# ioloizou/g1_locomotion

Hardware: AMD Instinct MI355X
Metric: QP solves/sec, SRBD N=10 12-state/12-input (higher is better)
Workload: dtype f64; 1 GPU; configs[1]: batch=4096/GPU random SRBD states, N=10, 2-contact alternating single support friction cone, fp64; tails deferred (SRBDQP_FLAG_DEFER_TAIL: the ~4 % of a batch that reach a rho-restart mark finish in the next launch on their stream; srbdqp_flush inside the timed region, every batch complete when the clock stops); steps rotate over 4 distinct device batches; horizon=10, batch_per_gpu=4096, kernel=wave_defer_f64_n10_s2, streams=2, longest_first_hint=False, deferred_tails=True, world_size=1, distinct_batches=4, max_iter=250, rho_restart_iter=0, rho_restart_count=0, set_up_dtype=f64

## Files before the change

g1_locomotion_amd/csrc/srbdqp_setup1.hpp:

```cpp
#pragma once
#include "srbdqp_split.hpp"

namespace srbdqp {

#ifdef SRBDQP_WAVE_STAMPS
#define WSTAMP(a, b, idx) SRBDQP_STAMP(a, b, idx)
#define WSTAMP_RT(a, b, idx) do { if ((a).stamps && threadIdx.x == 0) (a).stamps[(size_t)(b) * 16 + (idx)] = (long long)__builtin_amdgcn_s_memrealtime(); } while (0)
#else
#define WSTAMP(a, b, idx) do { } while (0)
#define WSTAMP_RT(a, b, idx) do { } while (0)
#endif

template <int N, int MAXS>
struct Setup1Smem {
    using S = CompactSmem<N, MAXS>;
    static constexpr int n = Dims<N>::n;
    static constexpr int up2(int v) { return (v + 1) & ~1; }
    static constexpr int o_x0 = S::o_x0, o_tm = S::o_tm, o_J = S::o_J;
    static constexpr int o_cp = S::o_R;
    static constexpr int o_mt = o_cp + up2(9 * N);
    static constexpr int o_ab = o_mt + 18 * N;
    static constexpr int o_gv = o_mt + up2(9 * S::NPAIR);
    static constexpr int o_t1 = o_gv + up2(9 * N);
    static constexpr int o_t2 = o_t1 + up2(9 * N);
    static constexpr int o_x0c = o_t1;
    static constexpr int o_tf = o_x0c + up2(S::nmax) + 16;
    static constexpr int endT = (o_t2 + up2(9 * N) > o_tf + 6 * N) ? o_t2 + up2(9 * N) : o_tf + 6 * N;
    static constexpr int o_xref = up2(endT);
    static constexpr int o_foot = o_xref + up2(N * 13);
    static constexpr int o_pcom = o_foot + N * 12;
    static constexpr int o_eh = o_foot;
    static constexpr int o_gx = o_foot;
    static constexpr int o_scr = o_xref;
    static constexpr int endIn = o_pcom + up2(N * 3);
    static constexpr int endIn2 = (endIn > o_scr + 258) ? endIn : o_scr + 258;
    static constexpr int kStgRow = 18;
    static constexpr int kStgTile = 16 * kStgRow;
    static constexpr int endStg = (endIn2 > o_cp + S::NT * kStgTile) ? endIn2 : o_cp + S::NT * kStgTile;
    static constexpr int endAb = o_ab + 16 * S::NT * kAbStride;
    static constexpr int o_end = endStg > endAb ? endStg : endAb;
    static constexpr size_t bytes = (size_t)o_end * sizeof(double);
    static constexpr int kPairs = S::NPAIR;
    static constexpr int kPairSlots = (N / 2) * N + N;
    static constexpr int o_pd = o_t1;
    static constexpr int o_pq = up2(endIn);
    static constexpr bool pairs_fit = N % 2 == 0 && kPairs <= 64 && 2 * kPairSlots <= 2 * up2(9 * N) && o_pq + 4 * kPairSlots <= o_end;
    static constexpr bool supported = SplitWs<N, MAXS>::supported && S::NT <= 4;
    static_assert(!supported || pairs_fit, "a lane and an LDS slot for every step pair of a horizon the one-wave kernel takes");
    static_assert(n + 6 * N <= o_end - o_eh || true, "");
};

template <int N, int MAXS, bool FUSED, bool DUMP, bool PHI, int RP>
__device__ __forceinline__ bool setup1_pass(const KArgs& a, const QpIo& io, const int b, double* sm, double& rho_b, int& rs_pass, int& rs_done) {
    using S = CompactSmem<N, MAXS>;
    using W = SplitWs<N, MAXS>;
    using L1 = Setup1Smem<N, MAXS>;
    constexpr int n = Dims<N>::n, m = Dims<N>::m, NT = S::NT;
    int lane = threadIdx.x;
    if constexpr (RP == 2) asm volatile("" : "+v"(lane));
    [[maybe_unused]] double* const park = sm + L1::o_end;
    int mcol = lane & 15, kq = lane >> 4;
    double* ws = FUSED ? nullptr : a.ws + (size_t)b * W::doubles;
    int* icnt = reinterpret_cast<int*>(sm + S::o_int);
    int* imisc = icnt + 2 * N;
    uint8_t* act = reinterpret_cast<uint8_t*>(imisc + 8);
    uint8_t* sct = reinterpret_cast<uint8_t*>(sm + S::o_ct);
    const double* SQ = sm + S::o_sq;
    const double* CP = sm + L1::o_cp;

    WSTAMP(a, b, 0);
    WSTAMP_RT(a, b, 12);
    constexpr int JT = (12 * N + 63) / 64;
    double yc, ys;
    [[maybe_unused]] double v_xr[JT];
    if constexpr (RP == 2) {
        const int k = lane < N ? lane : 0;
        yc = sm[S::o_tm + k * 9 + 0];
        ys = sm[S::o_tm + k * 9 + 1];
    } else {
        const double* gx0 = io.x0 + (size_t)b * 13;
        const double* gxr = io.xref + (size_t)b * N * 13;
        const double* gft = io.foot + (size_t)b * N * 12;
        const uint8_t* gct = io.contact + (size_t)b * N * 4;
        const double* gpc = io.pcom ? io.pcom + (size_t)b * N * 3 : nullptr;
        const double v_x0 = gx0[lane < 13 ? lane : 0];
        const uint8_t v_ct = gct[lane < 4 * N ? lane : 0];
        const double v_yaw = gxr[(lane < N ? lane : 0) * 13 + 2];
        double v_f[JT][3], v_p[JT][3];
#pragma unroll
        for (int t = 0; t < JT; ++t) {
            const int tt = (lane + 64 * t < 12 * N) ? lane + 64 * t : 0;
            const int k = tt / 12, ci = (tt % 12) / 3;
            const double* pc = gpc ? gpc + k * 3 : gxr + k * 13 + 3;
#pragma unroll
            for (int c = 0; c < 3; ++c) { v_f[t][c] = gft[k * 12 + 3 * ci + c]; v_p[t][c] = pc[c]; }
            v_xr[t] = gxr[k * 13 + (tt - 12 * k)];
        }
        sincos(v_yaw, &ys, &yc);
        if (lane < 13) sm[S::o_x0 + lane] = v_x0;
        if (lane >= 32 && lane < 44) sm[S::o_sq + lane - 32] = a.sqrtq[lane - 32];
        if (lane < N * 4) sct[lane] = v_ct ? 1 : 0;
        if (lane < N) {
            double* T = sm + S::o_tm + lane * 9;
            T[0] = yc;  T[1] = ys;  T[2] = 0.0;
            T[3] = -ys; T[4] = yc;  T[5] = 0.0;
            T[6] = 0.0; T[7] = 0.0; T[8] = 1.0;
        }
        {
            const bool flag = (lane < 4 * N) && v_ct != 0;
            const unsigned long long bal = __ballot(flag);
            if (flag) act[__popcll(bal & ((1ull << lane) - 1ull))] = (uint8_t)lane;
            if (lane < N) icnt[lane] = __popcll(bal & ((4 * (lane + 1) >= 64) ? ~0ull : ((1ull << (4 * (lane + 1))) - 1ull)));
            const bool over = lane < N && __popcll((bal >> (4 * (lane < N ? lane : 0))) & 0xFull) > MAXS;
            const unsigned long long viol = __ballot(over);
            if (lane == 0) {
                imisc[0] = __popcll(bal);
                imisc[1] = viol != 0ull;
                sm[S::o_misc] = 0.0;
                sm[S::o_misc + 1] = 0.0;
            }
        }
#pragma unroll
        for (int t = 0; t < JT; ++t) {
            const int tt = lane + 64 * t;
            const int k = (tt < 12 * N ? tt : 0) / 12, cc = tt - 12 * k, ax = cc % 3;
            const double cs = __shfl(yc, k), sn = __shfl(ys, k);
            const double i0 = a.iinv[0], i1 = a.iinv[1], i2 = a.iinv[2];
            const double w00 = cs * cs * i0 + sn * sn * i1, w01 = cs * sn * (i0 - i1), w11 = sn * sn * i0 + cs * cs * i1;
            const double rx = v_f[t][0] - v_p[t][0];
            const double ry = v_f[t][1] - v_p[t][1];
            const double rz = v_f[t][2] - v_p[t][2];
            const double s0 = (ax == 0) ? 0.0 : ((ax == 1) ? -rz : ry);
            const double s1 = (ax == 0) ? rz : ((ax == 1) ? 0.0 : -rx);
            const double s2 = (ax == 0) ? -ry : ((ax == 1) ? rx : 0.0);
            if (tt < 12 * N) {
                double* J = sm + S::o_J + k * 36;
                J[0 * 12 + cc] = w00 * s0 + w01 * s1;
                J[1 * 12 + cc] = w01 * s0 + w11 * s1;
                J[2 * 12 + cc] = i2 * s2;
            }
        }
    }
    double ccm = 0.0, csm = 0.0;
#pragma unroll
    for (int k = 0; k < N; ++k) {
        const double c = lane_bcast(yc, k), s = lane_bcast(ys, k);
        ccm += (k <= lane) ? c : 0.0;
        csm += (k <= lane) ? s : 0.0;
    }
    if (lane < N) {
        double* C = sm + L1::o_cp + lane * 9;
        C[0] = ccm;  C[1] = csm; C[2] = 0.0;
        C[3] = -csm; C[4] = ccm; C[5] = 0.0;
        C[6] = 0.0;  C[7] = 0.0; C[8] = (double)(lane + 1);
    }
    __syncthreads();
    const int na = imisc[0];
    const int n_eff = 3 * na;
    double* xs0 = sm + L1::o_mt;
    static_assert(L1::o_end - L1::o_mt >= n + 12 * N, "early-exit scratch");
    if (RP != 2 && (imisc[1] != 0 || na == 0)) {
        if constexpr (DUMP) { if (lane == 0) a.ub_out[(size_t)b * m] = (imisc[1] != 0) ? -1.0 : 0.0; return false; }
        for (int c = lane; c < n; c += 64) xs0[c] = 0.0;
        if (io.y_out) for (int i = lane; i < m; i += 64) io.y_out[(size_t)b * m + i] = 0.0;
        if (lane == 0) {
            if (io.status) io.status[b] = (imisc[1] != 0) ? kStatusContactBound : 1;
            if (io.iters) io.iters[b] = a.iters_base;
            if constexpr (!FUSED) ws[S::o_misc + 1] = 1.0;
        }
        __syncthreads();
        rollout_and_store_to<N, S, 64>(a, io.u_out, io.x_out, b, sm, xs0, xs0 + n);
        return false;
    }

    WSTAMP(a, b, 1);
    const double dt = a.dt, dt2 = a.dt * a.dt, dtm = a.dt * a.inv_mass, dt2m = dt2 * a.inv_mass;
    double* DE = sm + L1::o_mt;
    double* GV = sm + L1::o_gv;
    if constexpr (RP != 2) {
#pragma unroll
        for (int t = 0; t < JT; ++t) {
            const int k = lane + 64 * t;
            const int kc = k < n ? k : 0, i = kc / 12, kk = kc - 12 * i;
            const double v = SQ[kk] * (free_response_sel<N, L1>(a, sm, i, kk) - v_xr[t]);
            if (k < n) sm[L1::o_eh + k] = v;
        }
    }
    const int pair_c = lane < L1::kPairs ? lane : L1::kPairs - 1;
    const int pair_r = pair_c / (N + 1), pair_k = pair_c - pair_r * (N + 1);
    const bool pair_lo = pair_k < N - pair_r;
    const int pair_m = pair_lo ? pair_r : N - 1 - pair_r, pair_i = pair_m + (pair_lo ? pair_k : pair_k - (N - pair_r));
    const double pair_da = CP[9 * pair_i] - CP[9 * pair_m], pair_db = CP[9 * pair_i + 1] - CP[9 * pair_m + 1];
    double* PD = sm + L1::o_pd;
    double* PQ = sm + L1::o_pq;
    {
        const double w0 = SQ[0] * SQ[0], w1 = SQ[1] * SQ[1], w2 = SQ[2] * SQ[2];
        const double da = pair_da, db = pair_db, dz = (double)(pair_i - pair_m);
        if (lane < L1::kPairs) {
            PD[2 * lane] = da;
            PD[2 * lane + 1] = db;
            PQ[4 * lane] = fma(w0 * da, da, (w1 * db) * db);
            PQ[4 * lane + 1] = fma(w0 * da, db, -((w1 * db) * da));
            PQ[4 * lane + 2] = fma(w0 * db, db, (w1 * da) * da);
            PQ[4 * lane + 3] = (pair_i == N - 1) ? 0.0 : (w2 * dz) * dz;
        }
    }
    __syncthreads();
    const int pair_base = (2 * lane < N) ? lane * (N + 1) : (N - lane) * N;
    if (lane < N) {
        const int mm = lane;
        double t1a = 0.0, t1b = 0.0, t2aa = 0.0, t2ab = 0.0, t2bb = 0.0, t2zz = 0.0;
#pragma unroll
        for (int s = 0; s < N; ++s) {
            if (s < N - mm) {
                const double* pd = PD + 2 * (pair_base + s);
                const double* pq = PQ + 4 * (pair_base + s);
                t1a += pd[0];
                t1b += pd[1];
                t2aa += pq[0];
                t2ab += pq[1];
                t2bb += pq[2];
                t2zz += pq[3];
            }
        }
        const double dzl = (double)(N - 1 - mm);
        t2zz = fma((SQ[2] * SQ[2]) * dzl, dzl, t2zz);
        const double t1z = (double)(((N - mm) * (N - mm - 1)) / 2);
        const double Cm[9] = {ccm, csm, 0.0, -csm, ccm, 0.0, 0.0, 0.0, (double)(mm + 1)};
        const double t1[9] = {t1a, t1b, 0.0, -t1b, t1a, 0.0, 0.0, 0.0, t1z};
        const double t2[9] = {t2aa, t2ab, 0.0, t2ab, t2bb, 0.0, 0.0, 0.0, t2zz};
        de_step<N>(Cm, t1, t2, SQ, dt2, mm, DE + 18 * mm);
    }
    auto gt_tables = [&](const double* vec) {
        {
            const double* v = vec + 12 * pair_i;
            const double p0 = SQ[0] * v[0], p1 = SQ[1] * v[1], p2 = SQ[2] * v[2], dz = (double)(pair_i - pair_m);
            if (lane < L1::kPairs) {
                PQ[4 * lane] = fma(dt, SQ[6] * v[6], dt2 * fma(pair_da, p0, (-pair_db) * p1));
                PQ[4 * lane + 1] = fma(dt, SQ[7] * v[7], dt2 * fma(pair_db, p0, pair_da * p1));
                PQ[4 * lane + 2] = fma(dt, SQ[8] * v[8], dt2 * (dz * p2));
            }
        }
        __syncthreads();
        if (lane < 3 * N) {
            const int j = lane / 3, comp = lane - 3 * j;
            const double* pq = PQ + 4 * ((2 * j < N) ? j * (N + 1) : (N - j) * N) + comp;
            double acc = 0.0;
#pragma unroll
            for (int s = 0; s < N; ++s)
                if (s < N - j) acc += pq[4 * s];
            GV[9 * j + comp] = acc;
        }
        static_assert(6 * N <= 64, "the force entries of the G'v tables are one trip of the wave");
        if (lane < 6 * N) {
            const int j = lane / 6, comp = 3 + (lane - 6 * j);
            const double* v = vec + 12 * j + ((comp < 6) ? comp : 3 + comp);
            const double winc = (comp < 6) ? 1.0 : 0.0;
            double acc = 0.0, w = (comp < 6) ? 0.0 : 1.0;
#pragma unroll
            for (int s = 0; s < N; ++s) {
                if (s < N - j) {
                    double term = w * v[12 * s];
                    asm volatile("" : "+v"(term));
                    acc += term;
                }
                w += winc;
            }
            GV[9 * j + comp] = acc;
        }
    };
    auto gt_eval = [&](int c) -> double {
        const int e = c / 3, ax = c - 3 * e, gc = act[e], j = gc >> 2;
        const double* J = sm + S::o_J + j * 36 + 3 * (gc & 3) + ax;
        const double* g = GV + 9 * j;
        return a.s * (J[0] * g[0] + J[12] * g[1] + J[24] * g[2] + SQ[3 + ax] * dt2m * g[3 + ax] + SQ[9 + ax] * dtm * g[6 + ax]);
    };
    __syncthreads();
    if constexpr (RP != 2) gt_tables(sm + L1::o_eh);
    __syncthreads();
    WSTAMP(a, b, 2);
    if constexpr (RP != 2) for (int c = lane; c < n_eff; c += 64) sm[S::o_q + c] = gt_eval(c);
    if (RP >= 2 || a.warm_u) {
        double* TF = sm + L1::o_tf;
        for (int c = lane; c < n_eff; c += 64)
            sm[L1::o_x0c + c] = (RP >= 2 ? park[c] : a.warm_u[(size_t)b * n + 3 * act[c / 3] + (c % 3)]) / a.s;
        __syncthreads();
        for (int tt = lane; tt < 6 * N; tt += 64) {
            const int j = tt / 6, comp = tt - 6 * j;
            double acc = 0.0;
            for (int e = (j ? icnt[j - 1] : 0); e < icnt[j]; ++e) {
                const double* x = sm + L1::o_x0c + 3 * e;
                if (comp < 3) {
                    const double* J = sm + S::o_J + j * 36 + comp * 12 + 3 * (act[e] & 3);
                    acc += J[0] * x[0] + J[1] * x[1] + J[2] * x[2];
                } else {
                    acc += x[comp - 3];
                }
            }
            TF[tt] = acc;
        }
        __syncthreads();
        for (int k = lane; k < n; k += 64) {
            const int i = k / 12, kk = k - 12 * i;
            const double acc = gx_row<N>(CP, TF, i, kk, dt, dt2, dtm, dt2m);
            sm[L1::o_gx + k] = SQ[kk] * a.s * acc;
        }
        __syncthreads();
        gt_tables(sm + L1::o_gx);
        __syncthreads();
        for (int c = lane; c < n_eff; c += 64) sm[S::o_px0 + c] = gt_eval(c) + a.rs2 * sm[L1::o_x0c + c];
    } else {
        for (int c = lane; c < n_eff; c += 64) sm[S::o_px0 + c] = 0.0;
    }

    if constexpr (PHI) {
        double* phi = ws + W::o_phi;
        const double x0_keep = (lane < 13) ? sm[S::o_x0 + lane] : 0.0;
        for (int kc = 0; kc < 13; ++kc) {
            __syncthreads();
            if (lane < 13) sm[S::o_x0 + lane] = (lane == kc) ? 1.0 : 0.0;
            __syncthreads();
            for (int k = lane; k < n; k += 64) {
                const int i = k / 12, kk = k - 12 * i;
                sm[L1::o_eh + k] = SQ[kk] * free_response<N, L1>(a, sm, i, kk);
            }
            __syncthreads();
            gt_tables(sm + L1::o_eh);
            __syncthreads();
            for (int c = lane; c < n_eff; c += 64) phi[c * 13 + kc] = gt_eval(c);
        }
        __syncthreads();
        if (lane < 13) sm[S::o_x0 + lane] = x0_keep;
        __syncthreads();
    }
    WSTAMP(a, b, 3);
    v4d Kt[NT][NT];
    __syncthreads();
    {
        double* AB = sm + L1::o_ab;
        kasm_rows<N>(sm + S::o_J, CP, DE, SQ, act, n_eff, a.s, dt2m, dtm, AB, lane, 64, 16 * NT);
        __syncthreads();
        typedef double d2 __attribute__((ext_vector_type(2)));
        const double dgxy = uni(a.rs2 + a.sigma + 2.0 * rho_b), dgz = uni(a.rs2 + a.sigma + (4.0 * a.mu * a.mu + a.rho_fz) * rho_b);
        const int d3 = (mcol - kq + 3) % 3;
        const double ind[3] = {d3 == 0 ? 1.0 : 0.0, d3 == 1 ? 1.0 : 0.0, d3 == 2 ? 1.0 : 0.0};
        double eqd[4];
#pragma unroll
        for (int q = 0; q < 4; ++q) eqd[q] = (kq + 4 * q == mcol) ? 1.0 : 0.0;
        double Bv[NT][8], dcol[NT];
#pragma unroll
        for (int tb = 0; tb < NT; ++tb) {
            const int c = 16 * tb + mcol;
            const d2* row = reinterpret_cast<const d2*>(AB + kAbStride * c + 8);
#pragma unroll
            for (int i = 0; i < 4; ++i) { const d2 v = row[i]; Bv[tb][2 * i] = v[0]; Bv[tb][2 * i + 1] = v[1]; }
            dcol[tb] = (c < n_eff) ? (((tb + mcol) % 3 < 2) ? dgxy : dgz) : 1.0;
        }
#pragma unroll
        for (int ta = 0; ta < NT; ++ta) {
#pragma unroll
            for (int q = 0; q < 4; ++q) {
                const int r = 16 * ta + kq + 4 * q;
                const d2* row = reinterpret_cast<const d2*>(AB + kAbStride * r);
                double Av[8];
#pragma unroll
                for (int i = 0; i < 4; ++i) { const d2 v = row[i]; Av[2 * i] = v[0]; Av[2 * i + 1] = v[1]; }
#pragma unroll
                for (int tb = ta; tb < NT; ++tb) {
                    double v = Av[0] * Bv[tb][0];
#pragma unroll
                    for (int i = 1; i < 6; ++i) v = fma(Av[i], Bv[tb][i], v);
                    const double ft = fma(Av[7], Bv[tb][7], Av[6] * Bv[tb][6]);
                    v = fma(ind[((ta + q - tb) % 3 + 3) % 3], ft, v);
                    if (ta == tb) v = fma(eqd[q], dcol[tb], v);
                    Kt[ta][tb][q] = v;
                }
            }
        }
    }
    __syncthreads();
    WSTAMP(a, b, 4);
    WSTAMP(a, b, 5);
    if constexpr (DUMP) {
        dump_presolved<N>(a, b, n_eff, na, sm + S::o_q, act, [&](auto&& put) {
#pragma unroll
            for (int ta = 0; ta < NT; ++ta)
#pragma unroll
                for (int tb = ta; tb < NT; ++tb)
#pragma unroll
                    for (int q = 0; q < 4; ++q)
                        if (16 * ta + kq + 4 * q <= 16 * tb + mcol) put(16 * ta + kq + 4 * q, 16 * tb + mcol, Kt[ta][tb][q]);
        });
        return false;
    }

    double* scr = sm + L1::o_scr;
    auto a_operand_read = [&](double (&op)[4]) {
#pragma unroll
        for (int r = 0; r < 4; ++r) op[r] = scr[mcol * 16 + ((4 * r + kq) ^ mcol)];
        asm volatile("" ::: "memory");
    };
    auto a_operand = [&](const v4d& x, double (&op)[4]) {
        asm volatile("" ::: "memory");
#pragma unroll
        for (int q = 0; q < 4; ++q) {
            const int row = kq + 4 * q;
            scr[row * 16 + (mcol ^ row)] = x[q];
        }
        asm volatile("" ::: "memory");
        a_operand_read(op);
    };
    const v4d zero4 = (v4d){0.0, 0.0, 0.0, 0.0};

    bool all_ok = true;
#pragma unroll
    for (int j = 0; j < NT; ++j) {
        bool ok;
        const v4d w = diag16_invert_dpp_packed(Kt[j][j], lane, ok, scr);
        all_ok = all_ok && ok;
        Kt[j][j] = w;
        if (j + 1 < NT) {
            double wa[4];
            a_operand_read(wa);
#pragma unroll
            for (int bb = j + 1; bb < NT; ++bb) {
                v4d o = zero4;
#pragma unroll
                for (int r = 0; r < 4; ++r) o = mfma_f64(wa[r], Kt[j][bb][r], o);
                Kt[j][bb] = o;
            }
#pragma unroll
            for (int aa = j + 1; aa < NT; ++aa)
#pragma unroll
                for (int bb = aa; bb < NT; ++bb)
#pragma unroll
                    for (int r = 0; r < 4; ++r) Kt[aa][bb] = mfma_f64(-Kt[j][aa][r], Kt[j][bb][r], Kt[aa][bb]);
        }
    }
    if (!all_ok && lane == 0) sm[S::o_misc] = 1.0;
    WSTAMP(a, b, 6);

#pragma unroll
    for (int i = 1; i < NT; ++i) {
        double wa[4];
        a_operand(Kt[i][i], wa);
#pragma unroll
        for (int j = 0; j < i; ++j) {
            v4d sacc = zero4;
#pragma unroll
            for (int k = j; k < i; ++k) {
                const v4d& wkj = (k == j) ? Kt[j][j] : Kt[j][k];
#pragma unroll
                for (int r = 0; r < 4; ++r) sacc = mfma_f64(Kt[k][i][r], wkj[r], sacc);
            }
            v4d o = zero4;
#pragma unroll
            for (int r = 0; r < 4; ++r) o = mfma_f64(-wa[r], sacc[r], o);
            Kt[j][i] = o;
        }
    }

    WSTAMP(a, b, 7);
    double kin[W::KS];
    if constexpr (!FUSED) {
        for (int i = lane; i < S::o_R; i += 64) ws[i] = sm[i];
        double* kinv = ws + W::o_kinv;
#pragma unroll
        for (int aa = 0; aa < NT; ++aa) {
#pragma unroll
            for (int bb = aa; bb < NT; ++bb) {
                v4d o = zero4;
#pragma unroll
                for (int k = bb; k < NT; ++k) {
                    const v4d& wka = (k == aa) ? Kt[aa][aa] : Kt[aa][k];
                    const v4d& wkb = (k == bb) ? Kt[bb][bb] : Kt[bb][k];
#pragma unroll
                    for (int r = 0; r < 4; ++r) o = mfma_f64(wka[r], wkb[r], o);
                }
                const int col = 16 * bb + mcol;
#pragma unroll
                for (int q = 0; q < 4; ++q) {
                    const int row = 16 * aa + kq + 4 * q;
                    if (row < n_eff && col < W::KS) kinv[row * W::KS + col] = (col < n_eff) ? o[q] : 0.0;
                    if (aa != bb && col < n_eff && row < W::KS) kinv[col * W::KS + row] = (row < n_eff) ? o[q] : 0.0;
                }
            }
        }
    } else {
        double* stg = sm + L1::o_cp;
        static_assert(L1::o_end - L1::o_cp >= NT * L1::kStgTile, "staging of one block column of K^-1");
        const int grp = lane >> 4;
        v4d Ku[NT][NT];
#pragma unroll
        for (int cb = NT - 1; cb >= 0; --cb) {
            asm volatile("" ::: "memory");
#pragma unroll
            for (int g = 0; g <= cb; ++g) {
                v4d o = zero4;
#pragma unroll
                for (int k = cb; k < NT; ++k) {
                    const v4d& wkg = (k == g) ? Kt[g][g] : Kt[g][k];
                    const v4d& wkc = (k == cb) ? Kt[cb][cb] : Kt[cb][k];
#pragma unroll
                    for (int r = 0; r < 4; ++r) o = mfma_f64(wkg[r], wkc[r], o);
                }
#pragma unroll
                for (int q = 0; q < 4; ++q) stg[g * L1::kStgTile + (kq + 4 * q) * L1::kStgRow + mcol] = o[q];
                if (g < cb) Ku[g][cb] = o;
            }
#pragma unroll
            for (int g = cb + 1; g < NT; ++g)
#pragma unroll
                for (int q = 0; q < 4; ++q) stg[g * L1::kStgTile + mcol * L1::kStgRow + kq + 4 * q] = Ku[cb][g][q];
            asm volatile("" ::: "memory");
            const double2* rowp = reinterpret_cast<const double2*>(stg + grp * L1::kStgTile + mcol * L1::kStgRow);
#pragma unroll
            for (int h = 0; h < 8; ++h) {
                if (16 * cb + 2 * h + 1 < W::KS + 1) {
                    const double2 v = rowp[h];
                    if (16 * cb + 2 * h < W::KS) kin[16 * cb + 2 * h] = v.x;
                    if (16 * cb + 2 * h + 1 < W::KS) kin[16 * cb + 2 * h + 1] = v.y;
                }
            }
            asm volatile("" ::: "memory");
        }
    }
    if constexpr (FUSED) {
        if (__builtin_amdgcn_readfirstlane(n_eff) < W::KS) {
#pragma unroll
            for (int c = 0; c < W::KS; ++c) kin[c] = (lane < n_eff && c < n_eff) ? kin[c] : 0.0;
        }
        __syncthreads();
        WSTAMP(a, b, 8);
        WSTAMP(a, b, 9);
        static_assert(L1::o_end >= SplitSmem<N, MAXS>::o_end, "the ADMM body's vectors live in this kernel's LDS");
        if constexpr (RP == 0) {
            admm_wave_body<N, MAXS>(a, b, rho_b, sm, kin);
        } else {
            WaveRestart rs;
            const int left = a.max_iter - rs_done;
            rs.pass = rs_pass;
            rs.more = rs_pass < a.restart_max && a.restart_every < left;
            rs.kcap = rs.more ? a.restart_every : left;
            rs.park = park;
            int status = -1, iters = 0;
            admm_wave_iterations<N, MAXS, true>(a, io, RP == 1 ? a.warm_u : nullptr, RP == 1 ? a.warm_y : nullptr, b, rho_b, sm, kin, sm + SplitSmem<N, MAXS>::o_xs,
                                                status, iters, &rs);
            rs_done += iters;
            if (status == 2 && rs.more) {
                rho_b = restart_rho_of(rho_b, rs.v);
                ++rs_pass;
                __syncthreads();
                return true;
            }
            admm_wave_finish<N, MAXS>(a, io, b, sm, status, rs_done);
        }
        WSTAMP(a, b, 10);
        WSTAMP(a, b, 11);
        WSTAMP_RT(a, b, 13);
    }
    return false;
}

template <int N, int MAXS, bool FUSED, bool DUMP = false, bool PHI = false, bool RST = false>
__global__ __launch_bounds__(64, 2) void srbdqp_setup1_kernel(KArgs a) {
    static_assert(!(PHI && FUSED), "dq/dx0 is a hand-over of the split pipeline");
    static_assert(!RST || (FUSED && !DUMP), "the restart in place belongs to the fused solve");
    static_assert(Setup1Smem<N, MAXS>::supported, "one wave holds all tiles: at most 4 x 4 tiles");
    static_assert(4 * N <= 64, "one ballot compacts the contact flags");
    extern __shared__ __attribute__((aligned(16))) double sm[];
    if ((int)blockIdx.x >= a.B) return;
    if (a.count_ptr && (int)blockIdx.x >= *a.count_ptr) return;
    const int b = SRBDQP_QP_INDEX(a);
    if (SRBDQP_RESTART_SKIP(a, b)) return;
    double rho_b = SRBDQP_RHO_OF(a, b);
    int rs_pass = 0, rs_done = 0;
    const QpIo io = io_of(a);
    if constexpr (!RST) {
        setup1_pass<N, MAXS, FUSED, DUMP, PHI, 0>(a, io, b, sm, rho_b, rs_pass, rs_done);
    } else {
        bool again = setup1_pass<N, MAXS, FUSED, DUMP, PHI, 1>(a, io, b, sm, rho_b, rs_pass, rs_done);
        if (!again) return;
        again = setup1_pass<N, MAXS, FUSED, DUMP, PHI, 2>(a, io, b, sm, rho_b, rs_pass, rs_done);
        if (!again) return;
        again = setup1_pass<N, MAXS, FUSED, DUMP, PHI, 2>(a, io, b, sm, rho_b, rs_pass, rs_done);
        if (!again) return;
        KArgs al = a;
        al.restart_max = 0;
        setup1_pass<N, MAXS, FUSED, DUMP, PHI, 2>(al, io, b, sm, rho_b, rs_pass, rs_done);
    }
}

__device__ __forceinline__ unsigned long long unis_u64(unsigned long long v) {
    int lo, hi;
    asm volatile("s_nop 1\n\tv_readfirstlane_b32 %0, %2\n\tv_readfirstlane_b32 %1, %3" : "=s"(lo), "=s"(hi) : "v"((int)(unsigned)v), "v"((int)(unsigned)(v >> 32)));
    return ((unsigned long long)(unsigned)hi << 32) | (unsigned long long)(unsigned)lo;
}
template <typename T> __device__ __forceinline__ T* unis_ptr(T* p) { return reinterpret_cast<T*>(unis_u64(reinterpret_cast<unsigned long long>(p))); }

__device__ __forceinline__ double* tail_claim(const KArgs& a) {
    int slot = 0;
    if (threadIdx.x == 0) slot = atomicAdd(a.tail_cnt + a.tail_iout, 1);
    slot = __builtin_amdgcn_readfirstlane(slot);
    if (slot >= a.tail_cap) return nullptr;
    return reinterpret_cast<double*>(a.tail_lists) + ((size_t)a.tail_iout * (size_t)a.tail_cap + (size_t)slot) * kTailRecDoubles;
}

__device__ __forceinline__ bool tail_export(const KArgs& a, const QpIo& io, int b, double rho_b, int rs_pass, int rs_done, const double* park) {
    const int lane = threadIdx.x;
    double* rec = tail_claim(a);
    if (!rec) return false;
    if (lane == 0) {
        TailRecHead* hd = reinterpret_cast<TailRecHead*>(rec);
        hd->b = b; hd->pass = rs_pass; hd->done = rs_done; hd->pad = 0; hd->rho = rho_b; hd->io = io;
        if (io.status) io.status[b] = kStatusPending;
    }
    rec[16 + lane] = park[lane]; rec[80 + lane] = park[64 + lane]; rec[144 + lane] = park[128 + lane];
    return true;
}

template <int N, int MAXS, bool FLUSH = false>
__global__ __launch_bounds__(64, 2) void srbdqp_wave_defer_kernel(KArgs a) {
    static_assert(Setup1Smem<N, MAXS>::supported && 4 * N <= 64, "the one-wave kernel's limits");
    extern __shared__ __attribute__((aligned(16))) double sm[];
    using L1 = Setup1Smem<N, MAXS>;
    const int lane = threadIdx.x;
    const int T = a.tail_wgs;
    double* const park = sm + L1::o_end;
    auto in_place = [&](const QpIo& io, const int b, double rho_b, int rs_pass, int rs_done) __attribute__((always_inline)) {
        bool again = setup1_pass<N, MAXS, true, false, false, 2>(a, io, b, sm, rho_b, rs_pass, rs_done);
        if (!again) return;
        again = setup1_pass<N, MAXS, true, false, false, 2>(a, io, b, sm, rho_b, rs_pass, rs_done);
        if (!again) return;
        KArgs al = a;
        al.restart_max = 0;
        setup1_pass<N, MAXS, true, false, false, 2>(al, io, b, sm, rho_b, rs_pass, rs_done);
    };
    if ((int)blockIdx.x < T) {
        const int i = blockIdx.x;
        int cnt = a.tail_cnt[a.tail_iin];
        cnt = cnt < a.tail_cap ? cnt : a.tail_cap;
        if (i == 0 && lane == 0) a.tail_cnt[a.tail_izero] = 0;
        const double* lin = reinterpret_cast<const double*>(a.tail_lists) + (size_t)a.tail_iin * (size_t)a.tail_cap * kTailRecDoubles;
        if (i >= cnt) return;
        const double* rec = lin + (size_t)i * kTailRecDoubles;
        const TailRecHead* hd = reinterpret_cast<const TailRecHead*>(rec);
        QpIo io;
        io.x0 = unis_ptr(hd->io.x0); io.xref = unis_ptr(hd->io.xref); io.foot = unis_ptr(hd->io.foot); io.pcom = unis_ptr(hd->io.pcom);
        io.contact = unis_ptr(hd->io.contact); io.u_out = unis_ptr(hd->io.u_out); io.x_out = unis_ptr(hd->io.x_out); io.y_out = unis_ptr(hd->io.y_out);
        io.status = unis_ptr(hd->io.status); io.iters = unis_ptr(hd->io.iters);
        const int b = __builtin_amdgcn_readfirstlane(hd->b);
        int rs_pass = __builtin_amdgcn_readfirstlane(hd->pass), rs_done = __builtin_amdgcn_readfirstlane(hd->done);
        double rho_b = unis(hd->rho);
        park[lane] = rec[16 + lane]; park[64 + lane] = rec[80 + lane]; park[128 + lane] = rec[144 + lane];
        __syncthreads();
        if (!setup1_pass<N, MAXS, true, false, false, 3>(a, io, b, sm, rho_b, rs_pass, rs_done)) return;
        if constexpr (!FLUSH) { if (tail_export(a, io, b, rho_b, rs_pass, rs_done, park)) return; }
        in_place(io, b, rho_b, rs_pass, rs_done);
    } else if constexpr (!FLUSH) {
        const int wg = (int)blockIdx.x - T;
        if (wg >= a.B) return;
        const int b = a.perm ? a.perm[wg] : wg;
        double rho_b = a.rho_qp ? a.rho_qp[b] : a.rho;
        int rs_pass = 0, rs_done = 0;
        const QpIo io = io_of(a);
        if (!setup1_pass<N, MAXS, true, false, false, 1>(a, io, b, sm, rho_b, rs_pass, rs_done)) return;
        if (tail_export(a, io, b, rho_b, rs_pass, rs_done, park)) return;
        in_place(io, b, rho_b, rs_pass, rs_done);
    }
}

}
```

Before: 40.80 million QP/s.

## Compute K inverse via backward substitution from LDL factors, dropping explicit triangular inverse

The blocked factorization now keeps a unit-upper factor scaled by the inverted diagonal blocks and stores W*W on the diagonal. K^-1 is then built column block by column block with a Takahashi-style backward recurrence (X_g = D_g^-1 - sum U_gl X_l). This replaces the separate triangular-inverse pass followed by an explicit product. The goal is fewer MFMA operations in setup, paid for with extra LDS transposes of the already-computed blocks in each column step. The non-fused path is folded into the same loop.

```diff
diff --git a/g1_locomotion_amd/csrc/srbdqp_setup1.hpp b/g1_locomotion_amd/csrc/srbdqp_setup1.hpp
--- a/g1_locomotion_amd/csrc/srbdqp_setup1.hpp
+++ b/g1_locomotion_amd/csrc/srbdqp_setup1.hpp
@@ -400,16 +400,6 @@
         for (int r = 0; r < 4; ++r) op[r] = scr[mcol * 16 + ((4 * r + kq) ^ mcol)];
         asm volatile("" ::: "memory");
     };
-    auto a_operand = [&](const v4d& x, double (&op)[4]) {
-        asm volatile("" ::: "memory");
-#pragma unroll
-        for (int q = 0; q < 4; ++q) {
-            const int row = kq + 4 * q;
-            scr[row * 16 + (mcol ^ row)] = x[q];
-        }
-        asm volatile("" ::: "memory");
-        a_operand_read(op);
-    };
     const v4d zero4 = (v4d){0.0, 0.0, 0.0, 0.0};
 
     bool all_ok = true;
@@ -418,7 +408,6 @@
         bool ok;
         const v4d w = diag16_invert_dpp_packed(Kt[j][j], lane, ok, scr);
         all_ok = all_ok && ok;
-        Kt[j][j] = w;
         if (j + 1 < NT) {
             double wa[4];
             a_operand_read(wa);
@@ -435,94 +424,82 @@
                 for (int bb = aa; bb < NT; ++bb)
 #pragma unroll
                     for (int r = 0; r < 4; ++r) Kt[aa][bb] = mfma_f64(-Kt[j][aa][r], Kt[j][bb][r], Kt[aa][bb]);
-        }
+#pragma unroll
+            for (int l = j + 1; l < NT; ++l) {
+                v4d o = zero4;
+#pragma unroll
+                for (int r = 0; r < 4; ++r) o = mfma_f64(-Kt[j][l][r], w[r], o);
+                Kt[j][l] = o;
+            }
+        }
+        v4d pj = zero4;
+#pragma unroll
+        for (int r = 0; r < 4; ++r) pj = mfma_f64(w[r], w[r], pj);
+        Kt[j][j] = pj;
     }
     if (!all_ok && lane == 0) sm[S::o_misc] = 1.0;
     WSTAMP(a, b, 6);
-
-#pragma unroll
-    for (int i = 1; i < NT; ++i) {
-        double wa[4];
-        a_operand(Kt[i][i], wa);
-#pragma unroll
-        for (int j = 0; j < i; ++j) {
-            v4d sacc = zero4;
-#pragma unroll
-            for (int k = j; k < i; ++k) {
-                const v4d& wkj = (k == j) ? Kt[j][j] : Kt[j][k];
-#pragma unroll
-                for (int r = 0; r < 4; ++r) sacc = mfma_f64(Kt[k][i][r], wkj[r], sacc);
-            }
-            v4d o = zero4;
-#pragma unroll
-            for (int r = 0; r < 4; ++r) o = mfma_f64(-wa[r], sacc[r], o);
-            Kt[j][i] = o;
-        }
-    }
-
     WSTAMP(a, b, 7);
+
     double kin[W::KS];
-    if constexpr (!FUSED) {
-        for (int i = lane; i < S::o_R; i += 64) ws[i] = sm[i];
-        double* kinv = ws + W::o_kinv;
-#pragma unroll
-        for (int aa = 0; aa < NT; ++aa) {
-#pragma unroll
-            for (int bb = aa; bb < NT; ++bb) {
-                v4d o = zero4;
-#pragma unroll
-                for (int k = bb; k < NT; ++k) {
-                    const v4d& wka = (k == aa) ? Kt[aa][aa] : Kt[aa][k];
-                    const v4d& wkb = (k == bb) ? Kt[bb][bb] : Kt[bb][k];
-#pragma unroll
-                    for (int r = 0; r < 4; ++r) o = mfma_f64(wka[r], wkb[r], o);
-                }
-                const int col = 16 * bb + mcol;
-#pragma unroll
-                for (int q = 0; q < 4; ++q) {
-                    const int row = 16 * aa + kq + 4 * q;
-                    if (row < n_eff && col < W::KS) kinv[row * W::KS + col] = (col < n_eff) ? o[q] : 0.0;
-                    if (aa != bb && col < n_eff && row < W::KS) kinv[col * W::KS + row] = (row < n_eff) ? o[q] : 0.0;
-                }
-            }
-        }
-    } else {
+    {
+        if constexpr (!FUSED) {
+            for (int i = lane; i < S::o_R; i += 64) ws[i] = sm[i];
+        }
         double* stg = sm + L1::o_cp;
         static_assert(L1::o_end - L1::o_cp >= NT * L1::kStgTile, "staging of one block column of K^-1");
-        const int grp = lane >> 4;
+        [[maybe_unused]] double* kinv = FUSED ? nullptr : ws + W::o_kinv;
+        [[maybe_unused]] const int grp = lane >> 4;
         v4d Ku[NT][NT];
 #pragma unroll
         for (int cb = NT - 1; cb >= 0; --cb) {
+            v4d Xc[NT];
             asm volatile("" ::: "memory");
 #pragma unroll
-            for (int g = 0; g <= cb; ++g) {
-                v4d o = zero4;
-#pragma unroll
-                for (int k = cb; k < NT; ++k) {
-                    const v4d& wkg = (k == g) ? Kt[g][g] : Kt[g][k];
-                    const v4d& wkc = (k == cb) ? Kt[cb][cb] : Kt[cb][k];
-#pragma unroll
-                    for (int r = 0; r < 4; ++r) o = mfma_f64(wkg[r], wkc[r], o);
+            for (int l = cb + 1; l < NT; ++l)
+#pragma unroll
+                for (int q = 0; q < 4; ++q) stg[l * L1::kStgTile + mcol * L1::kStgRow + kq + 4 * q] = Ku[cb][l][q];
+            asm volatile("" ::: "memory");
+#pragma unroll
+            for (int l = cb + 1; l < NT; ++l)
+#pragma unroll
+                for (int q = 0; q < 4; ++q) Xc[l][q] = stg[l * L1::kStgTile + (kq + 4 * q) * L1::kStgRow + mcol];
+            asm volatile("" ::: "memory");
+#pragma unroll
+            for (int g = cb; g >= 0; --g) {
+                v4d o = (g == cb) ? Kt[cb][cb] : zero4;
+#pragma unroll
+                for (int l = g + 1; l < NT; ++l)
+#pragma unroll
+                    for (int r = 0; r < 4; ++r) o = mfma_f64(Kt[g][l][r], Xc[l][r], o);
+                Xc[g] = o;
+                if (g < cb) Ku[g][cb] = o;
+                if constexpr (FUSED) {
+#pragma unroll
+                    for (int q = 0; q < 4; ++q) stg[g * L1::kStgTile + (kq + 4 * q) * L1::kStgRow + mcol] = o[q];
+                } else {
+                    const int col = 16 * cb + mcol;
+#pragma unroll
+                    for (int q = 0; q < 4; ++q) {
+                        const int row = 16 * g + kq + 4 * q;
+                        if (row < n_eff && col < W::KS) kinv[row * W::KS + col] = (col < n_eff) ? o[q] : 0.0;
+                        if (g != cb && col < n_eff && row < W::KS) kinv[col * W::KS + row] = (row < n_eff) ? o[q] : 0.0;
+                    }
                 }
-#pragma unroll
-                for (int q = 0; q < 4; ++q) stg[g * L1::kStgTile + (kq + 4 * q) * L1::kStgRow + mcol] = o[q];
-                if (g < cb) Ku[g][cb] = o;
-            }
-#pragma unroll
-            for (int g = cb + 1; g < NT; ++g)
-#pragma unroll
-                for (int q = 0; q < 4; ++q) stg[g * L1::kStgTile + mcol * L1::kStgRow + kq + 4 * q] = Ku[cb][g][q];
-            asm volatile("" ::: "memory");
-            const double2* rowp = reinterpret_cast<const double2*>(stg + grp * L1::kStgTile + mcol * L1::kStgRow);
-#pragma unroll
-            for (int h = 0; h < 8; ++h) {
-                if (16 * cb + 2 * h + 1 < W::KS + 1) {
-                    const double2 v = rowp[h];
-                    if (16 * cb + 2 * h < W::KS) kin[16 * cb + 2 * h] = v.x;
-                    if (16 * cb + 2 * h + 1 < W::KS) kin[16 * cb + 2 * h + 1] = v.y;
+            }
+            if constexpr (FUSED) {
+                asm volatile("" ::: "memory");
+                const double2* rowp = reinterpret_cast<const double2*>(stg + grp * L1::kStgTile + mcol * L1::kStgRow);
+#pragma unroll
+                for (int h = 0; h < 8; ++h) {
+                    if (16 * cb + 2 * h + 1 < W::KS + 1) {
+                        const double2 v = rowp[h];
+                        if (16 * cb + 2 * h < W::KS) kin[16 * cb + 2 * h] = v.x;
+                        if (16 * cb + 2 * h + 1 < W::KS) kin[16 * cb + 2 * h + 1] = v.y;
+                    }
                 }
-            }
-            asm volatile("" ::: "memory");
+                asm volatile("" ::: "memory");
+            }
         }
     }
     if constexpr (FUSED) {
```

Result: faster. 42.12 million QP/s, median of 6 (+3.2%).
